# Varghese-Kuruvilla/Visual-Odometry-pipeline

Measured on NVIDIA B200. Metric: frame-pairs/sec (match+PnP), higher is better.
Workload: dtype tf32x3 / f32+f64 PnP

## Files before the change

### visual-odometry-pipeline_b200/csrc/match_f32_tc.cu

```cuda
#include "common.cuh"
#include "tc_ptx.cuh"
#include <cuda_fp16.h>
#include <stdlib.h>

#ifndef VO_TC_DBG
#define VO_TC_DBG 0
#endif
#ifndef VO_TC_PERSIST_MAX_TILES
#define VO_TC_PERSIST_MAX_TILES 64
#endif

namespace vo {
namespace {

constexpr int TC_BM = 128;
constexpr int TC_BN = 128;
constexpr int TC_D = 128;
constexpr int TC_KB = 32;
constexpr int TC_NKB = TC_D / TC_KB;
constexpr int TC_EXT_K = 8;
template <int PASSES>
struct TcCfg {
    static constexpr bool F8 = PASSES == 8 || PASSES == 9;
    static constexpr bool TOP1 = PASSES == 9;
    static constexpr bool K256 = F8;
    static constexpr bool F16 = PASSES == 16 || K256;
    static constexpr int KBOX = F8 ? 128 : 64;
    static constexpr bool H16 = F16 || PASSES == 48;
    static constexpr bool THREE = PASSES == 3 || PASSES == 48;
    static constexpr bool ALLWARP_COLS = PASSES == 48;
    static constexpr int KDIM = K256 ? 256 : TC_D;
    static constexpr bool SINGLE = !THREE;
    static constexpr int ALO = H16 ? 64 : TC_D;
    static constexpr int BN = F16 ? 192 : (SINGLE ? 160 : 128);
    static constexpr int STAGES = F16 ? 9 : (SINGLE ? 10 : 13);
    static constexpr int BLOCK_BYTES = BN * 128;
    static constexpr int TMEM_A = K256 ? 384 : (F16 ? 416 : (SINGLE ? 384 : 256));
    static constexpr int TMEM_EXT = F16 ? 384 : 320;
    static constexpr int OFF_SCOL = STAGES * BLOCK_BYTES;
    static constexpr int SCOL_N = F16 ? 0 : (ALLWARP_COLS ? 2 * 4 * BN : 2 * 2 * 4 * BN);
    static constexpr int OFF_ROW2 = OFF_SCOL + SCOL_N * 8;
    static constexpr int OFF_BAR = OFF_ROW2 + (H16 ? 4 * TC_BM * 4 : 0);
    static constexpr int SMEM_BYTES = OFF_BAR + 512 + 1024;
    static_assert(SMEM_BYTES <= 232448, "dynamic shared memory of one CTA (227 KB)");
    static constexpr uint32_t IDESC = (1u << 4) | (2u << 7) | (2u << 10) | ((uint32_t)(BN >> 3) << 17) | ((uint32_t)(TC_BM >> 4) << 24);
    static constexpr uint32_t IDESC16 = (1u << 4) | ((uint32_t)(BN >> 3) << 17) | ((uint32_t)(TC_BM >> 4) << 24);
    static constexpr float ACC_SCALE = PASSES == 48 ? 1.0f / 65536.0f : 1.0f;
};
constexpr int TC_THREADS = 576;
constexpr int TC_WARP_TMA = 16, TC_WARP_MMA = 17;
constexpr int TC_TMEM_COLS = 512;
constexpr int TC_CLUSTER = 2;

using namespace tc;



__global__ void __launch_bounds__(256)
prep_kernel(const float *__restrict__ x, long long rows, float *__restrict__ hi, float *__restrict__ lo,
            float *__restrict__ norm2, float *__restrict__ ext) {
    const long long row = (long long)blockIdx.x * 8 + (threadIdx.x >> 5);
    if (row >= rows) return;
    const int lane = threadIdx.x & 31;
    const float4 v = reinterpret_cast<const float4 *>(x)[row * 32 + lane];
    float4 h = make_float4(to_tf32(v.x), to_tf32(v.y), to_tf32(v.z), to_tf32(v.w));
    reinterpret_cast<float4 *>(hi)[row * 32 + lane] = h;
    if (lo) {
        float4 l = make_float4(to_tf32(v.x - h.x), to_tf32(v.y - h.y), to_tf32(v.z - h.z), to_tf32(v.w - h.w));
        reinterpret_cast<float4 *>(lo)[row * 32 + lane] = l;
    }
    if (norm2) {
        float s = __fadd_rn(__fadd_rn(__fmul_rn(v.x, v.x), __fmul_rn(v.y, v.y)), __fadd_rn(__fmul_rn(v.z, v.z), __fmul_rn(v.w, v.w)));
#pragma unroll
        for (int o = 16; o > 0; o >>= 1) s = __fadd_rn(s, __shfl_xor_sync(0xffffffffu, s, o));
        if (lane == 0) norm2[row] = s;
        if (ext) {
            float4 e = make_float4(0.f, 0.f, 0.f, 0.f);
            if (lane == 0) {
                const float n1 = to_tf32(s), n2 = to_tf32(__fsub_rn(s, n1));
                const float n3 = to_tf32(__fsub_rn(__fsub_rn(s, n1), n2));
                e = make_float4(-n1, -n2, -n3, 0.f);
            }
            if (lane < TC_EXT_K / 4) reinterpret_cast<float4 *>(ext)[row * (TC_EXT_K / 4) + lane] = e;
        }
    }
}

__global__ void __launch_bounds__(256)
prep16_kernel(const float *__restrict__ x, long long rows, __half *__restrict__ h16, float *__restrict__ norm2,
              float *__restrict__ ext) {
    const long long row = (long long)blockIdx.x * 8 + (threadIdx.x >> 5);
    if (row >= rows) return;
    const int lane = threadIdx.x & 31;
    const float4 v = reinterpret_cast<const float4 *>(x)[row * 32 + lane];
    const __half2 p0 = __floats2half2_rn(v.x, v.y), p1 = __floats2half2_rn(v.z, v.w);
    uint2 w;
    w.x = *reinterpret_cast<const uint32_t *>(&p0);
    w.y = *reinterpret_cast<const uint32_t *>(&p1);
    reinterpret_cast<uint2 *>(h16)[row * 32 + lane] = w;
    if (norm2) {
        float s = __fadd_rn(__fadd_rn(__fmul_rn(v.x, v.x), __fmul_rn(v.y, v.y)), __fadd_rn(__fmul_rn(v.z, v.z), __fmul_rn(v.w, v.w)));
#pragma unroll
        for (int o = 16; o > 0; o >>= 1) s = __fadd_rn(s, __shfl_xor_sync(0xffffffffu, s, o));
        if (lane == 0) norm2[row] = s;
        if (ext) {
// ... 193 lines not shown
                    s1 = gt ? sc[j0 + j] : s1;
                }
                thr = fmaxf(thr, s1);
            } else {
#pragma unroll
                for (int j = 0; j < 4; ++j) row_insert(sc[j0 + j], cbase + j0 + j, s1, s2, i1, i2);
                thr = fmaxf(thr, s2);
            }
        }
    }
}

template <bool EXT, bool F8>
__device__ __noinline__ void tc_a_to_tmem(const uint8_t *src, bool have, int k0, int row_elems, bool a_warp, bool ones_warp,
                                          uint32_t taddr_a, uint32_t taddr_ext, uint32_t bar_a, uint32_t wait_bar,
                                          uint32_t wait_parity, int lane) {
    constexpr int EPV = F8 ? 16 : 8;
    float v[32];
    if (a_warp) {
#pragma unroll
        for (int k = 0; k < 8; ++k) {
            uint4 x = (have && k0 + k * EPV < row_elems) ? __ldg(reinterpret_cast<const uint4 *>(src) + k) : make_uint4(0, 0, 0, 0);
            uint32_t wd[4] = {x.x, x.y, x.z, x.w};
#pragma unroll
            for (int i = 0; i < 4; ++i) {
                if (EXT) {
                    const __half2 d = __hmul2(*reinterpret_cast<const __half2 *>(&wd[i]), __floats2half2_rn(2.0f, 2.0f));
                    wd[i] = *reinterpret_cast<const uint32_t *>(&d);
                }
                v[4 * k + i] = __uint_as_float(wd[i]);
            }
        }
    }
    if (wait_bar) {
        tc::mbar_wait(wait_bar, wait_parity);
        tc::tc_fence_after();
    }
    if (a_warp) {
        tc::tc_st32(taddr_a, v);
        asm volatile("tcgen05.wait::st.sync.aligned;" ::: "memory");
        tc::tc_fence_before();
        if (lane == 0) tc::mbar_arrive(bar_a);
    }
    if (EXT && ones_warp) {
        const float ones[8] = {1.f, 1.f, 1.f, 0.f, 0.f, 0.f, 0.f, 0.f};
        tc::tc_st8(taddr_ext, ones);
        asm volatile("tcgen05.wait::st.sync.aligned;" ::: "memory");
        tc::tc_fence_before();
        if (lane == 0) tc::mbar_arrive(bar_a);
    }
}

template <int PASSES, int METRIC, bool COLS, bool PERSIST_T = false>
__global__ void __cluster_dims__(TC_CLUSTER, 1, 1) __launch_bounds__(TC_THREADS, 1)
match_f32_tc_kernel(const __grid_constant__ CUtensorMap map_b_hi, const __grid_constant__ CUtensorMap map_b_lo,
                    const float *__restrict__ a_hi, const float *__restrict__ a_lo, int n_stride, int m_stride,
                    const int32_t *__restrict__ n_ref, const int32_t *__restrict__ n_cur,
                    const float *__restrict__ row_norm, const float *__restrict__ col_norm, int n_split,
                    vo_row_partial *__restrict__ part, unsigned long long *__restrict__ colkey,
                    long long *__restrict__ dbg, int pair_group, int row_elems, int lgrid_x, int n_pairs) {
    extern __shared__ uint8_t smem_raw[];
    const uint32_t base = (smem_u32(smem_raw) + 1023u) & ~1023u;
    uint8_t *smem = smem_raw + (base - smem_u32(smem_raw));

    int b = blockIdx.z, rblock = blockIdx.x;
    if (pair_group > 1) {
        const int clusters_x = gridDim.x / TC_CLUSTER;
        const int set0 = (blockIdx.z / pair_group) * pair_group;
        const int gs = min(pair_group, (int)gridDim.z - set0);
        const int l = (blockIdx.z - set0) * clusters_x + (int)(blockIdx.x / TC_CLUSTER);
        b = set0 + l % gs;
        rblock = (l / gs) * TC_CLUSTER + (int)(blockIdx.x % TC_CLUSTER);
    }
    const int split = blockIdx.y;
    const int N = n_ref ? min(n_ref[b], n_stride) : n_stride;
    const int M = n_cur ? min(n_cur[b], m_stride) : m_stride;
    const int row0 = rblock * TC_BM;
    using Cfg = TcCfg<PASSES>;
    constexpr int BN = Cfg::BN, STAGES = Cfg::STAGES, BLOCK_BYTES = Cfg::BLOCK_BYTES, HALF = BN / 2;
    constexpr int TMEM_A = Cfg::TMEM_A, TMEM_EXT = Cfg::TMEM_EXT;
    constexpr uint32_t IDESC = Cfg::IDESC;
    const int tiles_total = (M + BN - 1) / BN;
    const int tiles_per_split = (tiles_total + n_split - 1) / n_split;
    const int t_begin = min(tiles_total, split * tiles_per_split);
    const int t_end = min(tiles_total, t_begin + tiles_per_split);
    const int n_tiles = t_end - t_begin;
    constexpr bool PERSIST = PERSIST_T;
    static_assert(!PERSIST || Cfg::F16, "only the fp16 / fp8 single passes have the item loop in their epilogue");
    struct Item { int b, row0, split, N, M, t_begin, n_tiles; };
    const int w_step = PERSIST ? (int)gridDim.x / TC_CLUSTER : 1;
    const int w_first = PERSIST ? (int)blockIdx.x / TC_CLUSTER : 0;
    const int w_end = PERSIST ? (lgrid_x / TC_CLUSTER) * n_split * n_pairs : 1;
    auto item_at = [&](int w) {
        Item I;
        if (!PERSIST) { I.b = b; I.row0 = row0; I.split = split; I.N = N; I.M = M; I.t_begin = t_begin; I.n_tiles = n_tiles; return I; }
        const int cx = lgrid_x / TC_CLUSTER;
        I.b = w / (cx * n_split);
        I.split = (w / cx) % n_split;
        I.row0 = ((w % cx) * TC_CLUSTER + (int)(blockIdx.x % TC_CLUSTER)) * TC_BM;
        I.N = n_ref ? min(n_ref[I.b], n_stride) : n_stride;
        I.M = n_cur ? min(n_cur[I.b], m_stride) : m_stride;
        const int tt = (I.M + BN - 1) / BN, tps = (tt + n_split - 1) / n_split;
        I.t_begin = min(tt, I.split * tps);
        I.n_tiles = min(tt, I.t_begin + tps) - I.t_begin;
        return I;
    };
    const int warp = threadIdx.x >> 5, lane = threadIdx.x & 31;
    const uint32_t crank = cluster_rank();
    const bool dbg_on = VO_TC_DBG && dbg != nullptr && rblock == 0 && blockIdx.y == 0 && b == 0;
    const long long t_kernel0 = dbg_on ? clock64() : 0;
    const bool trace_on = VO_TC_DBG && dbg != nullptr && dbg[15] == 1;
    const long long t_trace0 = (trace_on && threadIdx.x == 0) ? clock64() : 0;
#define TC_DBG_BEGIN() const long long _t0 = dbg_on ? clock64() : 0
#define TC_DBG_END(slot) do { if (dbg_on) dbg_acc[slot] += clock64() - _t0; } while (0)
    long long dbg_acc[4] = {0, 0, 0, 0};

    constexpr bool F16 = Cfg::F16;
    constexpr bool H16 = Cfg::H16, THREE = Cfg::THREE, SCALED = PASSES == 48;
    constexpr bool EXT = !THREE && (METRIC == VO_METRIC_L2);
    constexpr int NKB = H16 ? Cfg::KDIM / Cfg::KBOX : TC_NKB;
    constexpr int ITEMS = THREE ? 2 * NKB : (EXT ? NKB + 1 : NKB);
    const uint32_t s_b = base;
    float *scol_v = reinterpret_cast<float *>(smem + Cfg::OFF_SCOL);
    uint32_t *scol_b = reinterpret_cast<uint32_t *>(smem + Cfg::OFF_SCOL + Cfg::SCOL_N * 4);
    const uint32_t s_bar = base + Cfg::OFF_BAR;
    auto bar_full = [&](int s) { return s_bar + 8u * s; };
    auto bar_empty = [&](int s) { return s_bar + 8u * (STAGES + s); };
    const uint32_t bar_a = s_bar + 8u * (2 * STAGES);
    auto bar_tfull = [&](int g) { return s_bar + 8u * (2 * STAGES + 1 + g); };
    auto bar_tempty = [&](int g) { return s_bar + 8u * (2 * STAGES + 3 + g); };
    uint32_t *tmem_slot = reinterpret_cast<uint32_t *>(smem + Cfg::OFF_BAR + 8 * (2 * STAGES + 5));
    volatile float *srow2 = reinterpret_cast<volatile float *>(smem + Cfg::OFF_ROW2);
    if (Cfg::H16 && threadIdx.x < 4 * TC_BM) srow2[threadIdx.x] = -INFINITY;

    if (threadIdx.x == 0) {
        for (int s = 0; s < STAGES; ++s) {
            mbar_init(bar_full(s), 1);
            mbar_init(bar_empty(s), TC_CLUSTER);
        }
        mbar_init(bar_a, THREE ? 16 : (EXT ? 12 : 8));
        for (int g = 0; g < 2; ++g) { mbar_init(bar_tfull(g), 1); mbar_init(bar_tempty(g), H16 ? 16 : 8); }
        asm volatile("fence.mbarrier_init.release.cluster;" ::: "memory");
    }
    if (warp == TC_WARP_MMA) {
        asm volatile("tcgen05.alloc.cta_group::1.sync.aligned.shared::cta.b32 [%0], %1;" ::"r"(smem_u32(tmem_slot)),
                     "r"((uint32_t)TC_TMEM_COLS)
                     : "memory");
        asm volatile("tcgen05.relinquish_alloc_permit.cta_group::1.sync.aligned;" ::: "memory");
    }
    tc_fence_before();
    __syncthreads();
    cluster_sync_all();
    tc_fence_after();
    const uint32_t tmem_base = *tmem_slot;
    if (dbg_on && threadIdx.x == 0) dbg[14] = clock64() - t_kernel0;

    auto tile_of = [&](int lt) { return t_begin + lt; };

    if (warp == TC_WARP_TMA) {
        if (lane == 0) {
            int it = 0;
            for (int w = w_first; w < w_end; w += w_step) {
            const Item I = item_at(w);
            for (int lt = 0; lt < I.n_tiles; ++lt) {
                const int brow = I.b * m_stride + (I.t_begin + lt) * BN;
                for (int item = 0; item < ITEMS; ++item, ++it) {
                    const int stage = it % STAGES;
                    const uint32_t phase = (uint32_t)(it / STAGES) & 1u;
                    { TC_DBG_BEGIN(); mbar_wait(bar_empty(stage), phase ^ 1u); TC_DBG_END(0); }
                    const bool is_ext = EXT && item == NKB;
                    mbar_expect_tx(bar_full(stage), is_ext ? BN * TC_EXT_K * 4 : BLOCK_BYTES);
                    if ((uint32_t)(it & 1) == crank) {
                        const int kb = is_ext ? 0 : (THREE ? (item >> 1) : item);
                        const bool is_lo = is_ext || (THREE && (item & 1));
                        tma_load_2d_mc(s_b + stage * BLOCK_BYTES, is_lo ? &map_b_lo : &map_b_hi, kb * (H16 ? Cfg::KBOX : TC_KB), brow,
                                       bar_full(stage), (uint16_t)((1u << TC_CLUSTER) - 1u));
                    }
                }
            }
            }
            if (dbg_on) dbg[4] = dbg_acc[0];
        }
    } else if (warp == TC_WARP_MMA) {
        {
            uint32_t stage = 0, phase = 0, a_phase = 0;
            long long mma_wait_full = 0, mma_wait_tempty = 0, mma_wait_a = 0;
            int gt = 0;
            for (int w = w_first; w < w_end; w += w_step) {
            const Item I = item_at(w);
            if (I.n_tiles == 0) continue;
            { const long long _t0 = dbg_on ? clock64() : 0;
              mbar_wait(bar_a, a_phase);
              if (dbg_on) mma_wait_a += clock64() - _t0; }
            a_phase ^= 1u;
            tc_fence_after();
            for (int lt = 0; lt < I.n_tiles; ++lt, ++gt) {
                const int buf = gt & 1;
                const uint32_t use = (uint32_t)(gt >> 1);
                { const long long _t0 = dbg_on ? clock64() : 0;
                  mbar_wait(bar_tempty(buf), (use & 1u) ^ 1u);
                  if (dbg_on) mma_wait_tempty += clock64() - _t0; }
                tc_fence_after();
                const uint32_t d_tmem = tmem_base + (uint32_t)(buf * BN);
#pragma unroll
                for (int item = 0; item < ITEMS; ++item) {
                    { const long long _t0 = dbg_on ? clock64() : 0;
                      mbar_wait(bar_full(stage), phase);
                      if (dbg_on) mma_wait_full += clock64() - _t0; }
                    tc_fence_after();
                    if (elect_one()) {
                        const int kb = THREE ? (item >> 1) : item;
                        const bool is_lo = THREE && (item & 1);
                        const uint32_t b_lo32 = (((s_b + stage * BLOCK_BYTES) & 0x3ffffu) >> 4) | (1u << 16);
                        const uint32_t a_hi_t = tmem_base + (uint32_t)(TMEM_A + kb * TC_KB);
                        if (EXT && item == NKB) {
                            const uint64_t bdesc = ((uint64_t)TC_SDESC_HI_32B << 32) | (uint64_t)b_lo32;
                            tc_mma_tf32_ts(d_tmem, tmem_base + (uint32_t)TMEM_EXT, bdesc, IDESC, 1u);
                        } else
#pragma unroll
                        for (int k8 = 0; k8 < TC_KB / 8; ++k8) {
                            const uint64_t bdesc = ((uint64_t)TC_SDESC_HI << 32) | (uint64_t)(b_lo32 + k8 * 2);
                            const uint32_t ahi = a_hi_t + k8 * 8;
                            if (Cfg::F8) {
                                tc_mma_f8_ts(d_tmem, ahi, bdesc, Cfg::IDESC16, (item | k8) ? 1u : 0u);
                            } else if (F16) {
// ... 119 lines not shown
#undef TC_FOLD8
                srow2[cq * TC_BM + rr] = Cfg::TOP1 ? s1 : s2;
                if (edbg) dbg_acc[2] += clock64() - _tm0;
                ++gt;
            };
            for (int lt = 0; lt < n_t - 1; ++lt) tile(lt, false);
            if (n_t > 0) {
                bool waited = false;
                if (has_next) {
                    const Item Nx = item_at(w + w_step);
                    if (Nx.n_tiles > 0) {
                        a_put(Nx.b, Nx.row0, bar_tfull(gt & 1), (uint32_t)(gt >> 1) & 1u);
                        a_stored = waited = true;
                    }
                }
                tile(n_t - 1, waited);
            }
            if (edbg) t_between = clock64();
            if (METRIC == VO_METRIC_L2) {
                s1 = __fsub_rn(s1, na); s2 = __fsub_rn(s2, na);
            }
            {
                const Item I = item_at(w);
                if (I.row0 + rr < n_stride) {
                    const size_t at = ((size_t)I.b * (n_split * 4) + I.split * 4 + cq) * n_stride + I.row0 + rr;
                    if (Cfg::TOP1) {
                        vo_row_best q;
                        q.s1 = float_to_ordered(-s1); q.i1 = i1;
                        reinterpret_cast<vo_row_best *>(part)[at] = q;
                    } else {
                        vo_row_partial p;
                        p.s1 = float_to_ordered(-s1); p.s2 = float_to_ordered(-s2);
                        p.i1 = i1; p.i2 = i2;
                        part[at] = p;
                    }
                }
            }
            if (has_next) {
                srow2[cq * TC_BM + rr] = -INFINITY;
                asm volatile("bar.sync 1, 512;" ::: "memory");
            }
        }
        if (edbg && q == 0 && lane == 0 && cq < 2) { dbg[5 + cq] = dbg_acc[0]; dbg[7 + cq] = dbg_acc[1]; dbg[9 + cq] = dbg_acc[2]; if (cq == 1) dbg[13] = dbg_acc[3]; }
        } else if constexpr (Cfg::ALLWARP_COLS) {
        constexpr int QW = BN / 4;
        static_assert(QW == 32, "two 16-column reads per thread, one merged column per lane");
        const int cq = warp >> 2;
        const int q = warp & 3;
        const int row = row0 + q * 32 + lane;
        const bool row_ok = row < N;
        const bool partial_rows = row0 + TC_BM > N;
        const uint32_t lane_base = tmem_base + ((uint32_t)(q * 32) << 16);
        if (n_tiles > 0) {
            const __half *src = reinterpret_cast<const __half *>(cq < 2 ? a_hi : a_lo) +
                                ((size_t)b * n_stride + min(row, n_stride - 1)) * TC_D + (cq & 1) * 64;
            const bool have = row < n_stride;
            float v[32];
#pragma unroll
            for (int k = 0; k < 8; ++k) {
                const uint4 x = have ? __ldg(reinterpret_cast<const uint4 *>(src) + k) : make_uint4(0, 0, 0, 0);
                v[4 * k] = __uint_as_float(x.x); v[4 * k + 1] = __uint_as_float(x.y);
                v[4 * k + 2] = __uint_as_float(x.z); v[4 * k + 3] = __uint_as_float(x.w);
            }
            tc_st32(lane_base + (uint32_t)(TMEM_A + cq * 32), v);
            asm volatile("tcgen05.wait::st.sync.aligned;" ::: "memory");
            tc_fence_before();
            if (lane == 0) mbar_arrive(bar_a);
        }
        float s1 = -INFINITY, s2 = -INFINITY, thr = -INFINITY;
        int32_t i1 = -1, i2 = -1;
        const int rr = q * 32 + lane;
        const float *cn = (METRIC == VO_METRIC_L2) ? col_norm + (size_t)b * m_stride : nullptr;
        const float na = (METRIC == VO_METRIC_L2 && row_ok) ? row_norm[(size_t)b * n_stride + row] : 0.0f;
        const bool cn_vec = (METRIC == VO_METRIC_L2) && ((reinterpret_cast<uintptr_t>(cn) & 15u) == 0);
        for (int lt = 0; lt < n_tiles; ++lt) {
            const int buf = lt & 1;
            const uint32_t use = (uint32_t)(lt >> 1);
            const int tcol0 = tile_of(lt) * BN;
            const int col0 = tcol0 + cq * QW;
            const bool full_tile = tcol0 + BN <= M;
            float *tile_cv = scol_v + buf * 4 * BN;
            uint32_t *tile_cb = scol_b + buf * 4 * BN;
            float *my_cv = tile_cv + q * BN + cq * QW;
            uint32_t *my_cb = tile_cb + q * BN + cq * QW;
            { TC_DBG_BEGIN(); mbar_wait(bar_tfull(buf), use & 1u); TC_DBG_END(0); }
            tc_fence_after();
            const long long _tc0 = dbg_on ? clock64() : 0;
            const uint32_t taddr = lane_base + (uint32_t)(buf * BN + cq * QW);
            uint32_t ra[16], rb[16];
            tc_ld16_issue(taddr, ra);
            tc_ld16_issue(taddr + 16, rb);
            {
                const float tau = fmaxf(fmaxf(srow2[((cq + 1) & 3) * TC_BM + rr], srow2[((cq + 2) & 3) * TC_BM + rr]),
                                        srow2[((cq + 3) & 3) * TC_BM + rr]);
                thr = fmaxf(thr, row_threshold(s2, tau));
            }
            float colthr = -INFINITY;
            bool col_any = false;
            if (COLS) {
                const int c = col0 + lane;
                float cur_best = INFINITY;
                if (c < M) {
                    const unsigned long long key = *reinterpret_cast<const volatile unsigned long long *>(colkey + (size_t)b * m_stride + c);
                    cur_best = (key == ~0ull) ? -INFINITY : -ordered_to_float((uint32_t)(key >> 32));
                }
                colthr = -warp_max_f32(-cur_best);
                my_cb[lane] = 0u;
                __syncwarp();
            }
            tc_ld_wait16(ra);
            tc_ld_wait16(rb);
            tc_fence_before();
            if (lane == 0) mbar_arrive(bar_tempty(buf));
            if (dbg_on) dbg_acc[1] += clock64() - _tc0;
            const long long _tm0 = dbg_on ? clock64() : 0;
#define TC_FOLD16(BUF, J0, MASKC, MASKR)                                                                                   \
    _Pragma("unroll") for (int u = 0; u < 2; ++u) {                                                                        \
        float v[8];                                                                                                        \
        _Pragma("unroll") for (int i = 0; i < 8; ++i) v[i] = __uint_as_float(BUF[8 * u + i]);                              \
        epi_group8<METRIC, MASKC, MASKR, COLS, false, SCALED, true>(v, col0 + (J0) + 8 * u, M, row_ok, na, cn, cn_vec, lane, \
                                                                  my_cv + (J0) + 8 * u, my_cb + (J0) + 8 * u, s1, s2, i1,  \
                                                                  i2, thr, colthr, &col_any);                              \
    }
            if (full_tile && !partial_rows) {
                TC_FOLD16(ra, 0, false, false) TC_FOLD16(rb, 16, false, false)
            } else {
                TC_FOLD16(ra, 0, true, true) TC_FOLD16(rb, 16, true, true)
            }
#undef TC_FOLD16
            srow2[cq * TC_BM + rr] = s2;
            if (COLS) {
                uint32_t merge;
                asm volatile("{\n\t.reg .pred p, r;\n\tsetp.ne.u32 p, %1, 0;\n\tbar.red.or.pred r, %2, 128, p;\n\tselp.u32 %0, 1, 0, r;\n\t}"
                             : "=r"(merge)
                             : "r"((uint32_t)col_any), "r"(1 + cq)
                             : "memory");
                if (q == 0 && merge) {
                    const int j = cq * QW + lane;
                    const int col = tcol0 + j;
                    float best = -INFINITY;
                    int brow = -1;
#pragma unroll
                    for (int qq = 0; qq < 4; ++qq) {
                        const float val = tile_cv[qq * BN + j];
                        const uint32_t bal = tile_cb[qq * BN + j];
                        if (bal != 0u && val > best) { best = val; brow = qq * 32 + __ffs(bal) - 1; }
                    }
                    if (col < M && brow >= 0 && row0 + brow < N) {
                        const unsigned long long key =
                            ((unsigned long long)float_to_ordered(-best) << 32) | (unsigned long long)(uint32_t)(row0 + brow);
                        unsigned long long *dst = colkey + (size_t)b * m_stride + col;
                        if (key < *reinterpret_cast<volatile unsigned long long *>(dst)) atomicMin(dst, key);
                    }
                }
            }
            if (dbg_on) dbg_acc[2] += clock64() - _tm0;
        }
        if (dbg_on && q == 0 && lane == 0 && cq < 2) { dbg[5 + cq] = dbg_acc[0]; dbg[7 + cq] = dbg_acc[1]; dbg[9 + cq] = dbg_acc[2]; }
        if (METRIC == VO_METRIC_L2 && !COLS) {
            s1 = __fsub_rn(s1, na); s2 = __fsub_rn(s2, na);
        }
        if (row < n_stride) {
            vo_row_partial p;
            p.s1 = float_to_ordered(-s1); p.s2 = float_to_ordered(-s2);
            p.i1 = i1; p.i2 = i2;
            part[((size_t)b * (n_split * 4) + split * 4 + cq) * n_stride + row] = p;
        }
        } else {
        const int g = warp >> 3;
        const int h = (warp >> 2) & 1;
        const int q = warp & 3;
        const int row = row0 + q * 32 + lane;
        const bool row_ok = row < N;
        const bool partial_rows = row0 + TC_BM > N;
        const uint32_t lane_base = tmem_base + ((uint32_t)(q * 32) << 16);

        if (n_tiles > 0 && (g == 0 || THREE)) {
            const float *src = (g == 0 ? a_hi : a_lo) + ((size_t)b * n_stride + min(row, n_stride - 1)) * TC_D;
            const bool have = row < n_stride;
#pragma unroll 1
            for (int c = 2 * h; c < 2 * h + 2; ++c) {
                float v[32];
#pragma unroll
                for (int k = 0; k < 8; ++k) {
                    const float4 x = have ? __ldg(reinterpret_cast<const float4 *>(src + c * 32) + k) : make_float4(0, 0, 0, 0);
                    const float sc2 = EXT ? 2.0f : 1.0f;
                    v[4 * k] = sc2 * x.x; v[4 * k + 1] = sc2 * x.y; v[4 * k + 2] = sc2 * x.z; v[4 * k + 3] = sc2 * x.w;
                }
                tc_st32(lane_base + (uint32_t)(TMEM_A + g * TC_D + c * 32), v);
            }
            asm volatile("tcgen05.wait::st.sync.aligned;" ::: "memory");
            tc_fence_before();
            if (lane == 0) mbar_arrive(bar_a);
        }

        if (EXT && n_tiles > 0 && g == 1 && h == 0) {
            const float ones[8] = {1.f, 1.f, 1.f, 0.f, 0.f, 0.f, 0.f, 0.f};
            tc_st8(lane_base + (uint32_t)TMEM_EXT, ones);
            asm volatile("tcgen05.wait::st.sync.aligned;" ::: "memory");
            tc_fence_before();
            if (lane == 0) mbar_arrive(bar_a);
        }

        float s1 = -INFINITY, s2 = -INFINITY;
        float thr = -INFINITY;
        int32_t i1 = -1, i2 = -1;
        float *grp_cv = scol_v + g * 2 * 4 * BN;
        uint32_t *grp_cb = scol_b + g * 2 * 4 * BN;
        const float *cn = (METRIC == VO_METRIC_L2) ? col_norm + (size_t)b * m_stride : nullptr;
        const float na = (METRIC == VO_METRIC_L2 && row_ok) ? row_norm[(size_t)b * n_stride + row] : 0.0f;
        const bool cn_vec = (METRIC == VO_METRIC_L2) && ((reinterpret_cast<uintptr_t>(cn) & 15u) == 0);

        for (int lt = g; lt < n_tiles; lt += 2) {
            const int col0 = tile_of(lt) * BN;
            const uint32_t use = (uint32_t)(lt >> 1);
            const bool full_tile = col0 + BN <= M;
            float *tile_cv = grp_cv + (use & 1u) * 4 * BN;
            uint32_t *tile_cb = grp_cb + (use & 1u) * 4 * BN;
            float *my_cv = tile_cv + q * BN;
            uint32_t *my_cb = tile_cb + q * BN;
            { TC_DBG_BEGIN(); mbar_wait(bar_tfull(g), use & 1u); TC_DBG_END(0); }
            tc_fence_after();
            const long long _tc0 = dbg_on ? clock64() : 0;
            const uint32_t taddr = lane_base + (uint32_t)(g * BN);
            if (THREE) {
#define TC_EPI_LOOP(MASKC, MASKR)                                                                                          \
    _Pragma("unroll 1") for (int j0 = HALF * h; j0 < HALF * h + HALF; j0 += 8) {                                                 \
        uint32_t cur[8];                                                                                                   \
        tc_ld8_issue(taddr + j0, cur);                                                                                     \
        tc_ld_wait8(cur);                                                                                                  \
        float v[8];                                                                                                        \
        _Pragma("unroll") for (int i = 0; i < 8; ++i) v[i] = __uint_as_float(cur[i]);                                      \
        epi_group8<METRIC, MASKC, MASKR, COLS, EXT, SCALED>(v, col0 + j0, M, row_ok, na, cn, cn_vec, lane, my_cv + j0, my_cb + j0, \
                                                    s1, s2, i1, i2, thr);                                                       \
    }
                if (full_tile && !partial_rows) { TC_EPI_LOOP(false, false) } else { TC_EPI_LOOP(true, true) }
#undef TC_EPI_LOOP
            } else if (COLS) {
                uint32_t cur[8], nxt[8];
                tc_ld8_issue(taddr + HALF * h, cur);
                tc_ld_wait8(cur);
#define TC_EPI_LOOP(MASKC, MASKR)                                                                                          \
    _Pragma("unroll 1") for (int j0 = HALF * h; j0 < HALF * h + HALF; j0 += 8) {                                                 \
        const bool more = j0 + 8 < HALF * h + HALF;                                                                            \
        if (more) tc_ld8_issue(taddr + j0 + 8, nxt);                                                                       \
        float v[8];                                                                                                        \
        _Pragma("unroll") for (int i = 0; i < 8; ++i) v[i] = __uint_as_float(cur[i]);                                      \
        epi_group8<METRIC, MASKC, MASKR, COLS, EXT>(v, col0 + j0, M, row_ok, na, cn, cn_vec, lane, my_cv + j0, my_cb + j0, \
                                                    s1, s2, i1, i2, thr);                                                       \
        if (more) {                                                                                                        \
            tc_ld_wait8(nxt);                                                                                              \
            _Pragma("unroll") for (int i = 0; i < 8; ++i) cur[i] = nxt[i];                                                 \
        }                                                                                                                  \
    }
                if (full_tile && !partial_rows) { TC_EPI_LOOP(false, false) } else { TC_EPI_LOOP(true, true) }
#undef TC_EPI_LOOP
            } else {
                uint32_t bufa[16], bufb[16];
                tc_ld16_issue(taddr + HALF * h, bufa);
                tc_ld_wait16(bufa);
#define TC_FOLD16(BUF, J0, MASKC, MASKR)                                                                                   \
    _Pragma("unroll") for (int u = 0; u < 2; ++u) {                                                                        \
        float v[8];                                                                                                        \
        _Pragma("unroll") for (int i = 0; i < 8; ++i) v[i] = __uint_as_float(BUF[8 * u + i]);                              \
        epi_group8<METRIC, MASKC, MASKR, COLS, EXT>(v, col0 + (J0) + 8 * u, M, row_ok, na, cn, cn_vec, lane,               \
                                                    my_cv + (J0) + 8 * u, my_cb + (J0) + 8 * u, s1, s2, i1, i2, thr);           \
    }
#define TC_EPI_LOOP(MASKC, MASKR)                                                                                          \
    _Pragma("unroll 1") for (int j0 = HALF * h; j0 < HALF * h + HALF; j0 += 32) {                                          \
        const bool has_b = j0 + 16 < HALF * h + HALF;                  \
        if (has_b) tc_ld16_issue(taddr + j0 + 16, bufb);                                                                   \
        TC_FOLD16(bufa, j0, MASKC, MASKR)                                                                                  \
        if (has_b) {                                                                                                       \
            tc_ld_wait16(bufb);                                                                                            \
            const bool more = j0 + 32 < HALF * h + HALF;                                                                   \
            if (more) tc_ld16_issue(taddr + j0 + 32, bufa);                                                                \
            TC_FOLD16(bufb, j0 + 16, MASKC, MASKR)                                                                         \
            if (more) tc_ld_wait16(bufa);                                                                                  \
        }                                                                                                                  \
    }
                if (full_tile && !partial_rows) { TC_EPI_LOOP(false, false) } else { TC_EPI_LOOP(true, true) }
#undef TC_EPI_LOOP
#undef TC_FOLD16
            }
            tc_fence_before();
            if (lane == 0) mbar_arrive(bar_tempty(g));
            if (dbg_on) dbg_acc[1] += clock64() - _tc0;
            const long long _tm0 = dbg_on ? clock64() : 0;
            if (COLS) group_bar(1 + g);
            if (COLS && (h * 4 + q) * 32 < BN) {
                const int j = (h * 4 + q) * 32 + lane;
// ... 22 lines not shown
        if (row < n_stride) {
            vo_row_partial p;
            p.s1 = float_to_ordered(-s1); p.s2 = float_to_ordered(-s2);
            p.i1 = i1; p.i2 = i2;
            part[((size_t)b * (n_split * 4) + split * 4 + g * 2 + h) * n_stride + row] = p;
        }
        }
    }

    if (dbg_on && threadIdx.x == 0) dbg[0] = clock64() - t_kernel0;
    tc_fence_before();
    __syncthreads();
    cluster_sync_all();
    if (warp == TC_WARP_MMA) {
        asm volatile("tcgen05.dealloc.cta_group::1.sync.aligned.b32 %0, %1;" ::"r"(tmem_base), "r"((uint32_t)TC_TMEM_COLS)
                     : "memory");
    }
    if (trace_on && threadIdx.x == 0) {
        uint32_t smid;
        asm volatile("mov.u32 %0, %%smid;" : "=r"(smid));
        long long *t = dbg + 16 + 3 * ((size_t)(blockIdx.z * gridDim.y + blockIdx.y) * gridDim.x + blockIdx.x);
        t[0] = t_trace0; t[1] = clock64(); t[2] = smid;
    }
}

typedef CUresult (*PFN_encodeTiled)(CUtensorMap *, CUtensorMapDataType, cuuint32_t, void *, const cuuint64_t *,
                                    const cuuint64_t *, const cuuint32_t *, const cuuint32_t *, CUtensorMapInterleave,
                                    CUtensorMapSwizzle, CUtensorMapL2promotion, CUtensorMapFloatOOBfill);

int make_map(vo_ctx *ctx, CUtensorMap *map, const void *ptr, long long rows, int box_rows, int row_elems = TC_D,
             bool half = false, bool bytes = false, bool narrow = false) {
    PFN_encodeTiled fn = (PFN_encodeTiled)ctx->encode_tiled;
    const size_t esz = bytes ? 1 : (half ? 2 : 4);
    cuuint64_t dims[2] = {(cuuint64_t)row_elems, (cuuint64_t)rows};
    cuuint64_t strides[1] = {(cuuint64_t)row_elems * esz};
    cuuint32_t box[2] = {(cuuint32_t)((narrow ? 32 : 128) / esz), (cuuint32_t)box_rows};
    cuuint32_t estr[2] = {1, 1};
    CUresult r = fn(map, bytes ? CU_TENSOR_MAP_DATA_TYPE_UINT8 : (half ? CU_TENSOR_MAP_DATA_TYPE_FLOAT16 : CU_TENSOR_MAP_DATA_TYPE_FLOAT32), 2, (void *)ptr, dims, strides, box, estr,
                    CU_TENSOR_MAP_INTERLEAVE_NONE, narrow ? CU_TENSOR_MAP_SWIZZLE_32B : CU_TENSOR_MAP_SWIZZLE_128B, CU_TENSOR_MAP_L2_PROMOTION_L2_256B,
                    CU_TENSOR_MAP_FLOAT_OOB_FILL_NONE);
    if (r != CUDA_SUCCESS) {
        set_error("cuTensorMapEncodeTiled failed (CUresult %d)", (int)r);
        return VO_ERR_CUDA;
    }
    return VO_OK;
}

template <int PASSES, int METRIC, bool COLS, bool PERSIST>
int launch_tc_kern(vo_ctx *ctx, dim3 grid, const CUtensorMap &bh, const CUtensorMap &bl, const float *a_hi, const float *a_lo,
                   int n_stride, int m_stride, const int32_t *n_ref, const int32_t *n_cur, const float *row_norm,
                   const float *col_norm, int n_split, vo_row_partial *part, unsigned long long *colkey, cudaStream_t st,
                   int row_elems) {
    auto kern = match_f32_tc_kernel<PASSES, METRIC, COLS, PERSIST>;
    long long *dbg = nullptr;
    const size_t n_ctas = (size_t)grid.x * grid.y * grid.z;
    const bool trace = getenv("VO_TC_TRACE") != nullptr;
    if (VO_TC_DBG && (getenv("VO_TC_DEBUG") || trace)) {
        static long long *dbg_dev = nullptr;
        static size_t dbg_cap = 0;
        const size_t need = 16 + (trace ? 3 * n_ctas : 0);
        if (dbg_cap < need) {
            if (dbg_dev) VO_CUDA(cudaFree(dbg_dev));
            VO_CUDA(cudaMalloc(&dbg_dev, need * sizeof(long long)));
            dbg_cap = need;
        }
        VO_CUDA(cudaMemsetAsync(dbg_dev, 0, 16 * sizeof(long long), st));
        if (trace) {
            const long long one = 1;
            VO_CUDA(cudaMemcpyAsync(dbg_dev + 15, &one, sizeof(one), cudaMemcpyHostToDevice, st));
        }
        dbg = dbg_dev;
    }
    VO_CUDA(cudaFuncSetAttribute(kern, cudaFuncAttributeMaxDynamicSharedMemorySize, TcCfg<PASSES>::SMEM_BYTES));
    int pair_group = 1;
    if (TcCfg<PASSES>::ALLWARP_COLS && COLS && !getenv("VO_TC_NO_INTERLEAVE"))
        pair_group = (int)max(1ll, min(8ll, (64ll << 20) / ((long long)m_stride * TC_D * 4)));
    dim3 launch_grid = grid;
    if (PERSIST) {
        static int max_clusters = 0;
        if (max_clusters == 0) {
            cudaLaunchConfig_t cfg = {};
            cfg.gridDim = dim3(TC_CLUSTER * 64);
            cfg.blockDim = dim3(TC_THREADS);
            cfg.dynamicSmemBytes = TcCfg<PASSES>::SMEM_BYTES;
            cudaLaunchAttribute at;
            at.id = cudaLaunchAttributeClusterDimension;
            at.val.clusterDim.x = TC_CLUSTER; at.val.clusterDim.y = 1; at.val.clusterDim.z = 1;
            cfg.attrs = &at;
            cfg.numAttrs = 1;
            int n = 0;
            if (cudaOccupancyMaxActiveClusters(&n, kern, &cfg) != cudaSuccess || n <= 0) {
                (void)cudaGetLastError();
                n = ctx->sm_count / TC_CLUSTER;
            }
            max_clusters = n;
        }
        const long long items = (long long)(grid.x / TC_CLUSTER) * grid.y * grid.z;
        const long long clusters = items < max_clusters ? items : (long long)max_clusters;
        launch_grid = dim3((unsigned)(clusters * TC_CLUSTER), 1, 1);
    }
    kern<<<launch_grid, TC_THREADS, TcCfg<PASSES>::SMEM_BYTES, st>>>(bh, bl, a_hi, a_lo, n_stride, m_stride, n_ref, n_cur, row_norm, col_norm,
                                                  n_split, part, colkey, dbg, pair_group, row_elems, (int)grid.x, (int)grid.z);
    VO_LAUNCH_CHECK(ctx);
    if (dbg && trace) {
        VO_CUDA(cudaStreamSynchronize(st));
        long long *h = (long long *)malloc(3 * n_ctas * sizeof(long long));
        VO_CUDA(cudaMemcpy(h, dbg + 16, 3 * n_ctas * sizeof(long long), cudaMemcpyDeviceToHost));
        double busy = 0, gap = 0;
        long long n_gap = 0, max_gap = 0;
        for (int sm = 0; sm < 256; ++sm) {
            long long last_end = -1;
            for (;;) {
                long long best = -1;
                size_t bi = 0;
                for (size_t i = 0; i < n_ctas; ++i)
                    if (h[3 * i + 2] == sm && (last_end < 0 || h[3 * i] >= last_end) && (best < 0 || h[3 * i] < best)) {
                        best = h[3 * i];
                        bi = i;
                    }
                if (best < 0) break;
                if (last_end >= 0) { gap += (double)(best - last_end); ++n_gap; if (best - last_end > max_gap) max_gap = best - last_end; }
                busy += (double)(h[3 * bi + 1] - h[3 * bi]);
                last_end = h[3 * bi + 1];
            }
        }
        fprintf(stderr, "[vo tc trace] passes=%d ctas=%zu mean_cta_cycles=%.0f mean_gap_cycles=%.0f max_gap=%lld gaps=%lld\n", PASSES,
                n_ctas, busy / (double)n_ctas, n_gap ? gap / (double)n_gap : 0.0, max_gap, n_gap);
        free(h);
    } else if (dbg) {
// ... 53 lines not shown
    int rc;
    const bool f16 = passes == 16, h16 = passes == 16 || passes == 48, three = passes == 3 || passes == 48;
    const size_t esz = h16 ? sizeof(__half) : sizeof(float);
    const int row_elems = src_u8 ? src_u8 : TC_D;
    const bool ext = !three && l2;
    const size_t src_row_bytes = src_u8 ? (size_t)src_u8 : TC_D * sizeof(float);
    const bool chained = n_stride == m_stride && (n_stride & 3) == 0 && B > 0 && !getenv("VO_NO_CHAIN_PREP") &&
                         reinterpret_cast<const char *>(cur) == reinterpret_cast<const char *>(ref) + (size_t)n_stride * src_row_bytes;
    const long long rows_p = chained ? rows_a + n_stride : rows_a;
    const size_t per_a = (size_t)rows_p * row_elems * esz, per_b = chained ? 0 : (size_t)rows_b * row_elems * esz;
    if ((rc = ws_get(ctx, WS_SPLIT_A, per_a * (three ? 2 : 1), (void **)&split_a))) return rc;
    const size_t per_ext = (size_t)(chained ? rows_p : rows_b) * TC_EXT_K * sizeof(float);
    if ((rc = ws_get(ctx, WS_SPLIT_B, per_b * (three ? 2 : 1) + (ext ? per_ext : 0) + 16, (void **)&split_b))) return rc;
    const long long rows_a4 = (rows_a + 3) & ~3ll;
    if ((rc = ws_get(ctx, WS_NORMS, sizeof(float) * (size_t)(chained ? rows_p : rows_a4 + rows_b), (void **)&norms))) return rc;
    const size_t shift = (size_t)n_stride * row_elems * esz;
    float *a_hi = split_a, *a_lo = three ? reinterpret_cast<float *>(reinterpret_cast<char *>(split_a) + per_a) : nullptr;
    float *b_hi = chained ? reinterpret_cast<float *>(reinterpret_cast<char *>(a_hi) + shift) : split_b;
    float *b_lo = !three ? nullptr : (chained ? reinterpret_cast<float *>(reinterpret_cast<char *>(a_lo) + shift)
                                              : reinterpret_cast<float *>(reinterpret_cast<char *>(split_b) + per_b));
    float *x_ext = ext ? reinterpret_cast<float *>(reinterpret_cast<char *>(split_b) + per_b * (three ? 2 : 1)) : nullptr;
    float *b_ext = (ext && chained) ? x_ext + (size_t)n_stride * TC_EXT_K : x_ext;
    float *row_norm = norms, *col_norm = chained ? norms + n_stride : norms + rows_a4;

    VO_PROF(ctx, st, VO_STAGE_PREP);
    for (int side = 0; side < (chained ? 1 : 2); ++side) {
        const float *src = side ? cur : ref;
        const long long rows = side ? rows_b : rows_p;
        float *hi = side ? b_hi : a_hi, *lo = side ? b_lo : a_lo;
        float *nrm = l2 ? (side ? col_norm : row_norm) : nullptr;
        float *xe = (side || chained) ? x_ext : nullptr;
        const unsigned g8 = (unsigned)((rows + 7) / 8);
        if (passes == 48)
            prep16x3_kernel<<<g8, 256, 0, st>>>(src, rows, reinterpret_cast<__half *>(hi), reinterpret_cast<__half *>(lo), nrm);
        else if (f16 && src_u8 == 32)
            prep16_u8_kernel<32><<<(unsigned)((rows + 31) / 32), 256, 0, st>>>(reinterpret_cast<const uint8_t *>(src), rows, reinterpret_cast<__half *>(hi), side ? col_norm : row_norm, xe);
        else if (f16 && src_u8)
            prep16_u8_kernel<128><<<g8, 256, 0, st>>>(reinterpret_cast<const uint8_t *>(src), rows, reinterpret_cast<__half *>(hi), side ? col_norm : row_norm, xe);
        else if (f16)
            prep16_kernel<<<g8, 256, 0, st>>>(src, rows, reinterpret_cast<__half *>(hi), nrm, xe);
        else
            prep_kernel<<<g8, 256, 0, st>>>(src, rows, hi, lo, nrm, xe);
        VO_LAUNCH_CHECK(ctx);
    }

    CUtensorMap mbh, mbl;
    const int bn = three ? TcCfg<3>::BN : (f16 ? TcCfg<16>::BN : TcCfg<1>::BN);
    if ((rc = make_map(ctx, &mbh, b_hi, rows_b, bn, row_elems, h16))) return rc;
    if (ext) rc = make_map(ctx, &mbl, b_ext, rows_b, bn, TC_EXT_K, false, false, true);
    else rc = make_map(ctx, &mbl, three ? b_lo : b_hi, rows_b, bn, TC_D, h16);
    if (rc) return rc;

    const int row_blocks = ceil_div(n_stride, TC_BM);
    const int grid_x = ceil_div(row_blocks, TC_CLUSTER) * TC_CLUSTER;
    const int n_split = pick_split(ctx, B, grid_x, ceil_div(m_stride, bn), 4);
    vo_row_partial *part;
    if ((rc = ws_get(ctx, WS_ROWPART, sizeof(vo_row_partial) * (size_t)B * n_split * 4 * n_stride, (void **)&part))) return rc;
    dim3 grid(grid_x, n_split, B);
    VO_PROF(ctx, st, VO_STAGE_MATCH);
#define TC_ARGS ctx, grid, mbh, mbl, a_hi, a_lo, n_stride, m_stride, n_ref, n_cur, row_norm, col_norm, n_split, part, colkey, st
#define TC_PICK(P, MET) (need_cols ? launch_tc<P, MET, true>(TC_ARGS) : launch_tc<P, MET, false>(TC_ARGS))
    if (passes == 3) rc = l2 ? TC_PICK(3, VO_METRIC_L2) : TC_PICK(3, VO_METRIC_COSINE);
    else if (passes == 48) rc = l2 ? TC_PICK(48, VO_METRIC_L2) : TC_PICK(48, VO_METRIC_COSINE);
    else if (f16) rc = l2 ? launch_tc<16, VO_METRIC_L2, false>(TC_ARGS, row_elems) : launch_tc<16, VO_METRIC_COSINE, false>(TC_ARGS);
    else rc = l2 ? TC_PICK(1, VO_METRIC_L2) : TC_PICK(1, VO_METRIC_COSINE);
#undef TC_PICK
#undef TC_ARGS
    if (rc) return rc;
    *part_out = part;
    *n_split_out = n_split * 4;
    *row_norm_out = nullptr;
    return VO_OK;
}

int match_bits_tc(vo_ctx *ctx, const uint8_t *ref, const uint8_t *cur, int B, int n_stride, int m_stride, const int32_t *n_ref,
                  const int32_t *n_cur, int need_cols, int need_second, vo_row_partial **part_out, int *n_split_out,
                  unsigned long long *colkey, cudaStream_t st) {
    if (!ctx->tc_ready) {
        void *fn = nullptr;
        cudaDriverEntryPointQueryResult qres;
        VO_CUDA(cudaGetDriverEntryPoint("cuTensorMapEncodeTiled", &fn, cudaEnableDefault, &qres));
        if (qres != cudaDriverEntryPointSuccess || !fn) {
            set_error("cuTensorMapEncodeTiled is not available from this driver");
            return VO_ERR_UNSUPPORTED;
        }
        ctx->encode_tiled = fn;
        ctx->tc_ready = 1;
    }
    constexpr int KD = 256, BN = TcCfg<8>::BN;
    const long long rows_a = (long long)B * n_stride, rows_b = (long long)B * m_stride;
    uint8_t *a8, *b8;
    int rc;
    const bool chained = n_stride == m_stride && B > 0 && !getenv("VO_NO_CHAIN_PREP") && cur == ref + (size_t)n_stride * 32;
    const long long rows_p = chained ? rows_a + n_stride : rows_a;
    if ((rc = ws_get(ctx, WS_SPLIT_A, (size_t)rows_p * KD, (void **)&a8))) return rc;
    if (chained) b8 = a8 + (size_t)n_stride * KD;
    else if ((rc = ws_get(ctx, WS_SPLIT_B, (size_t)rows_b * KD, (void **)&b8))) return rc;
    VO_PROF(ctx, st, VO_STAGE_PREP);
    prep_bits8_kernel<<<(unsigned)((rows_p + 7) / 8), 256, 0, st>>>(ref, rows_p, a8);
    VO_LAUNCH_CHECK(ctx);
    if (!chained) {
        prep_bits8_kernel<<<(unsigned)((rows_b + 7) / 8), 256, 0, st>>>(cur, rows_b, b8);
        VO_LAUNCH_CHECK(ctx);
    }

    auto pass = [&](const uint8_t *A, const uint8_t *Bm, int ns, int ms, const int32_t *na, const int32_t *nb, int slot,
                    vo_row_partial **part, int *n_split, bool second) -> int {
        CUtensorMap map;
        int r;
        if ((r = make_map(ctx, &map, Bm, (long long)B * ms, BN, KD, false, true))) return r;
        const int row_blocks = ceil_div(ns, TC_BM);
        const int grid_x = ceil_div(row_blocks, TC_CLUSTER) * TC_CLUSTER;
        const int ns_split = pick_split(ctx, B, grid_x, ceil_div(ms, BN), 4);
        if ((r = ws_get(ctx, slot, sizeof(vo_row_partial) * (size_t)B * ns_split * 4 * ns, (void **)part))) return r;
        dim3 grid(grid_x, ns_split, B);
        *n_split = ns_split * 4;
        if (second)
            return launch_tc<8, VO_METRIC_COSINE, false>(ctx, grid, map, map, reinterpret_cast<const float *>(A), nullptr, ns, ms, na, nb,
                                                         nullptr, nullptr, ns_split, *part, nullptr, st, KD);
        return launch_tc<9, VO_METRIC_COSINE, false>(ctx, grid, map, map, reinterpret_cast<const float *>(A), nullptr, ns, ms, na, nb,
                                                     nullptr, nullptr, ns_split, *part, nullptr, st, KD);
    };
    VO_PROF(ctx, st, VO_STAGE_MATCH);
    if ((rc = pass(a8, b8, n_stride, m_stride, n_ref, n_cur, WS_ROWPART, part_out, n_split_out, need_second != 0))) return rc;
    if (need_cols) {
        vo_row_partial *part2;
        int n_split2;
        if ((rc = pass(b8, a8, m_stride, n_stride, n_cur, n_ref, WS_ROWPART2, &part2, &n_split2, false))) return rc;
        colkey_from_partials_kernel<<<dim3(ceil_div(m_stride, 256), B), 256, 0, st>>>(reinterpret_cast<const vo_row_best *>(part2), n_split2,
                                                                                      m_stride, n_cur, colkey);
        VO_LAUNCH_CHECK(ctx);
    }
    return VO_OK;
}

}
```

Before: 8371.

## Use 4-CTA TMA multicast clusters and all-warp epilogue for 3-pass TF32 matching

For the 3-pass (tf32x3) matcher, the thread-block cluster grows from 2 to 4 CTAs, so each B tile is loaded once by one CTA and multicast to four, cutting L2 traffic per CTA. The 3-pass path also moves to the all-warp epilogue with the A-fill layout generalized to fp32 chunks, and the interleave pair_group sizing now accounts for element width. Larger clusters can make scheduling harder, can pad more row blocks per pair, and make every stage slot wait for more consumers before it is freed.

```diff
diff --git a/visual-odometry-pipeline_b200/csrc/match_f32_tc.cu b/visual-odometry-pipeline_b200/csrc/match_f32_tc.cu
--- a/visual-odometry-pipeline_b200/csrc/match_f32_tc.cu
+++ b/visual-odometry-pipeline_b200/csrc/match_f32_tc.cu
@@ -5,6 +5,9 @@
 
 #ifndef VO_TC_DBG
 #define VO_TC_DBG 0
+#endif
+#ifndef VO_TC_CLUSTER3
+#define VO_TC_CLUSTER3 4
 #endif
 #ifndef VO_TC_PERSIST_MAX_TILES
 #define VO_TC_PERSIST_MAX_TILES 64
@@ -28,7 +31,8 @@
     static constexpr int KBOX = F8 ? 128 : 64;
     static constexpr bool H16 = F16 || PASSES == 48;
     static constexpr bool THREE = PASSES == 3 || PASSES == 48;
-    static constexpr bool ALLWARP_COLS = PASSES == 48;
+    static constexpr bool ALLWARP_COLS = THREE;
+    static constexpr bool ALLWARP = F16 || ALLWARP_COLS;
     static constexpr int KDIM = K256 ? 256 : TC_D;
     static constexpr bool SINGLE = !THREE;
     static constexpr int ALO = H16 ? 64 : TC_D;
@@ -40,17 +44,17 @@
     static constexpr int OFF_SCOL = STAGES * BLOCK_BYTES;
     static constexpr int SCOL_N = F16 ? 0 : (ALLWARP_COLS ? 2 * 4 * BN : 2 * 2 * 4 * BN);
     static constexpr int OFF_ROW2 = OFF_SCOL + SCOL_N * 8;
-    static constexpr int OFF_BAR = OFF_ROW2 + (H16 ? 4 * TC_BM * 4 : 0);
+    static constexpr int OFF_BAR = OFF_ROW2 + (ALLWARP ? 4 * TC_BM * 4 : 0);
     static constexpr int SMEM_BYTES = OFF_BAR + 512 + 1024;
     static_assert(SMEM_BYTES <= 232448, "dynamic shared memory of one CTA (227 KB)");
     static constexpr uint32_t IDESC = (1u << 4) | (2u << 7) | (2u << 10) | ((uint32_t)(BN >> 3) << 17) | ((uint32_t)(TC_BM >> 4) << 24);
     static constexpr uint32_t IDESC16 = (1u << 4) | ((uint32_t)(BN >> 3) << 17) | ((uint32_t)(TC_BM >> 4) << 24);
     static constexpr float ACC_SCALE = PASSES == 48 ? 1.0f / 65536.0f : 1.0f;
+    static constexpr int CLUSTER = PASSES == 3 ? VO_TC_CLUSTER3 : 2;
 };
 constexpr int TC_THREADS = 576;
 constexpr int TC_WARP_TMA = 16, TC_WARP_MMA = 17;
 constexpr int TC_TMEM_COLS = 512;
-constexpr int TC_CLUSTER = 2;
 
 using namespace tc;
 
@@ -350,7 +354,7 @@
 }
 
 template <int PASSES, int METRIC, bool COLS, bool PERSIST_T = false>
-__global__ void __cluster_dims__(TC_CLUSTER, 1, 1) __launch_bounds__(TC_THREADS, 1)
+__global__ void __cluster_dims__(TcCfg<PASSES>::CLUSTER, 1, 1) __launch_bounds__(TC_THREADS, 1)
 match_f32_tc_kernel(const __grid_constant__ CUtensorMap map_b_hi, const __grid_constant__ CUtensorMap map_b_lo,
                     const float *__restrict__ a_hi, const float *__restrict__ a_lo, int n_stride, int m_stride,
                     const int32_t *__restrict__ n_ref, const int32_t *__restrict__ n_cur,
@@ -358,6 +362,7 @@
                     vo_row_partial *__restrict__ part, unsigned long long *__restrict__ colkey,
                     long long *__restrict__ dbg, int pair_group, int row_elems, int lgrid_x, int n_pairs) {
     extern __shared__ uint8_t smem_raw[];
+    constexpr int TC_CLUSTER = TcCfg<PASSES>::CLUSTER;
     const uint32_t base = (smem_u32(smem_raw) + 1023u) & ~1023u;
     uint8_t *smem = smem_raw + (base - smem_u32(smem_raw));
 
@@ -429,7 +434,7 @@
     auto bar_tempty = [&](int g) { return s_bar + 8u * (2 * STAGES + 3 + g); };
     uint32_t *tmem_slot = reinterpret_cast<uint32_t *>(smem + Cfg::OFF_BAR + 8 * (2 * STAGES + 5));
     volatile float *srow2 = reinterpret_cast<volatile float *>(smem + Cfg::OFF_ROW2);
-    if (Cfg::H16 && threadIdx.x < 4 * TC_BM) srow2[threadIdx.x] = -INFINITY;
+    if (Cfg::ALLWARP && threadIdx.x < 4 * TC_BM) srow2[threadIdx.x] = -INFINITY;
 
     if (threadIdx.x == 0) {
         for (int s = 0; s < STAGES; ++s) {
@@ -437,7 +442,7 @@
             mbar_init(bar_empty(s), TC_CLUSTER);
         }
         mbar_init(bar_a, THREE ? 16 : (EXT ? 12 : 8));
-        for (int g = 0; g < 2; ++g) { mbar_init(bar_tfull(g), 1); mbar_init(bar_tempty(g), H16 ? 16 : 8); }
+        for (int g = 0; g < 2; ++g) { mbar_init(bar_tfull(g), 1); mbar_init(bar_tempty(g), Cfg::ALLWARP ? 16 : 8); }
         asm volatile("fence.mbarrier_init.release.cluster;" ::: "memory");
     }
     if (warp == TC_WARP_MMA) {
@@ -468,7 +473,7 @@
                     { TC_DBG_BEGIN(); mbar_wait(bar_empty(stage), phase ^ 1u); TC_DBG_END(0); }
                     const bool is_ext = EXT && item == NKB;
                     mbar_expect_tx(bar_full(stage), is_ext ? BN * TC_EXT_K * 4 : BLOCK_BYTES);
-                    if ((uint32_t)(it & 1) == crank) {
+                    if ((uint32_t)it % TC_CLUSTER == crank) {
                         const int kb = is_ext ? 0 : (THREE ? (item >> 1) : item);
                         const bool is_lo = is_ext || (THREE && (item & 1));
                         tma_load_2d_mc(s_b + stage * BLOCK_BYTES, is_lo ? &map_b_lo : &map_b_hi, kb * (H16 ? Cfg::KBOX : TC_KB), brow,
@@ -694,17 +699,22 @@
         const bool partial_rows = row0 + TC_BM > N;
         const uint32_t lane_base = tmem_base + ((uint32_t)(q * 32) << 16);
         if (n_tiles > 0) {
-            const __half *src = reinterpret_cast<const __half *>(cq < 2 ? a_hi : a_lo) +
-                                ((size_t)b * n_stride + min(row, n_stride - 1)) * TC_D + (cq & 1) * 64;
+            constexpr int CHUNKS = H16 ? 1 : 2;
+            static_assert(Cfg::ALO == 2 * CHUNKS * 32, "A_lo follows A_hi: quarter cq stores TMEM columns (cq * CHUNKS + c) * 32");
+            const uint8_t *src = reinterpret_cast<const uint8_t *>(cq < 2 ? a_hi : a_lo) +
+                                 ((size_t)b * n_stride + min(row, n_stride - 1)) * TC_D * (H16 ? 2 : 4) + (cq & 1) * CHUNKS * 128;
             const bool have = row < n_stride;
-            float v[32];
-#pragma unroll
-            for (int k = 0; k < 8; ++k) {
-                const uint4 x = have ? __ldg(reinterpret_cast<const uint4 *>(src) + k) : make_uint4(0, 0, 0, 0);
-                v[4 * k] = __uint_as_float(x.x); v[4 * k + 1] = __uint_as_float(x.y);
-                v[4 * k + 2] = __uint_as_float(x.z); v[4 * k + 3] = __uint_as_float(x.w);
-            }
-            tc_st32(lane_base + (uint32_t)(TMEM_A + cq * 32), v);
+#pragma unroll 1
+            for (int c = 0; c < CHUNKS; ++c) {
+                float v[32];
+#pragma unroll
+                for (int k = 0; k < 8; ++k) {
+                    const uint4 x = have ? __ldg(reinterpret_cast<const uint4 *>(src + c * 128) + k) : make_uint4(0, 0, 0, 0);
+                    v[4 * k] = __uint_as_float(x.x); v[4 * k + 1] = __uint_as_float(x.y);
+                    v[4 * k + 2] = __uint_as_float(x.z); v[4 * k + 3] = __uint_as_float(x.w);
+                }
+                tc_st32(lane_base + (uint32_t)(TMEM_A + (cq * CHUNKS + c) * 32), v);
+            }
             asm volatile("tcgen05.wait::st.sync.aligned;" ::: "memory");
             tc_fence_before();
             if (lane == 0) mbar_arrive(bar_a);
@@ -809,6 +819,7 @@
             part[((size_t)b * (n_split * 4) + split * 4 + cq) * n_stride + row] = p;
         }
         } else {
+        static_assert(PASSES == 1, "the other passes run an all-warp epilogue");
         const int g = warp >> 3;
         const int h = (warp >> 2) & 1;
         const int q = warp & 3;
@@ -817,8 +828,8 @@
         const bool partial_rows = row0 + TC_BM > N;
         const uint32_t lane_base = tmem_base + ((uint32_t)(q * 32) << 16);
 
-        if (n_tiles > 0 && (g == 0 || THREE)) {
-            const float *src = (g == 0 ? a_hi : a_lo) + ((size_t)b * n_stride + min(row, n_stride - 1)) * TC_D;
+        if (n_tiles > 0 && g == 0) {
+            const float *src = a_hi + ((size_t)b * n_stride + min(row, n_stride - 1)) * TC_D;
             const bool have = row < n_stride;
 #pragma unroll 1
             for (int c = 2 * h; c < 2 * h + 2; ++c) {
@@ -829,7 +840,7 @@
                     const float sc2 = EXT ? 2.0f : 1.0f;
                     v[4 * k] = sc2 * x.x; v[4 * k + 1] = sc2 * x.y; v[4 * k + 2] = sc2 * x.z; v[4 * k + 3] = sc2 * x.w;
                 }
-                tc_st32(lane_base + (uint32_t)(TMEM_A + g * TC_D + c * 32), v);
+                tc_st32(lane_base + (uint32_t)(TMEM_A + c * 32), v);
             }
             asm volatile("tcgen05.wait::st.sync.aligned;" ::: "memory");
             tc_fence_before();
@@ -865,20 +876,7 @@
             tc_fence_after();
             const long long _tc0 = dbg_on ? clock64() : 0;
             const uint32_t taddr = lane_base + (uint32_t)(g * BN);
-            if (THREE) {
-#define TC_EPI_LOOP(MASKC, MASKR)                                                                                          \
-    _Pragma("unroll 1") for (int j0 = HALF * h; j0 < HALF * h + HALF; j0 += 8) {                                                 \
-        uint32_t cur[8];                                                                                                   \
-        tc_ld8_issue(taddr + j0, cur);                                                                                     \
-        tc_ld_wait8(cur);                                                                                                  \
-        float v[8];                                                                                                        \
-        _Pragma("unroll") for (int i = 0; i < 8; ++i) v[i] = __uint_as_float(cur[i]);                                      \
-        epi_group8<METRIC, MASKC, MASKR, COLS, EXT, SCALED>(v, col0 + j0, M, row_ok, na, cn, cn_vec, lane, my_cv + j0, my_cb + j0, \
-                                                    s1, s2, i1, i2, thr);                                                       \
-    }
-                if (full_tile && !partial_rows) { TC_EPI_LOOP(false, false) } else { TC_EPI_LOOP(true, true) }
-#undef TC_EPI_LOOP
-            } else if (COLS) {
+            if (COLS) {
                 uint32_t cur[8], nxt[8];
                 tc_ld8_issue(taddr + HALF * h, cur);
                 tc_ld_wait8(cur);
@@ -1007,6 +1005,7 @@
                    const float *col_norm, int n_split, vo_row_partial *part, unsigned long long *colkey, cudaStream_t st,
                    int row_elems) {
     auto kern = match_f32_tc_kernel<PASSES, METRIC, COLS, PERSIST>;
+    constexpr int TC_CLUSTER = TcCfg<PASSES>::CLUSTER;
     long long *dbg = nullptr;
     const size_t n_ctas = (size_t)grid.x * grid.y * grid.z;
     const bool trace = getenv("VO_TC_TRACE") != nullptr;
@@ -1028,8 +1027,10 @@
     }
     VO_CUDA(cudaFuncSetAttribute(kern, cudaFuncAttributeMaxDynamicSharedMemorySize, TcCfg<PASSES>::SMEM_BYTES));
     int pair_group = 1;
-    if (TcCfg<PASSES>::ALLWARP_COLS && COLS && !getenv("VO_TC_NO_INTERLEAVE"))
-        pair_group = (int)max(1ll, min(8ll, (64ll << 20) / ((long long)m_stride * TC_D * 4)));
+    if (TcCfg<PASSES>::ALLWARP_COLS && COLS && !getenv("VO_TC_NO_INTERLEAVE")) {
+        const long long b_row_bytes = 2ll * TC_D * (TcCfg<PASSES>::H16 ? 2 : 4);
+        pair_group = (int)max(1ll, min(8ll, (64ll << 20) / ((long long)m_stride * b_row_bytes)));
+    }
     dim3 launch_grid = grid;
     if (PERSIST) {
         static int max_clusters = 0;
@@ -1189,7 +1190,8 @@
     if (rc) return rc;
 
     const int row_blocks = ceil_div(n_stride, TC_BM);
-    const int grid_x = ceil_div(row_blocks, TC_CLUSTER) * TC_CLUSTER;
+    const int cluster = passes == 3 ? TcCfg<3>::CLUSTER : 2;
+    const int grid_x = ceil_div(row_blocks, cluster) * cluster;
     const int n_split = pick_split(ctx, B, grid_x, ceil_div(m_stride, bn), 4);
     vo_row_partial *part;
     if ((rc = ws_get(ctx, WS_ROWPART, sizeof(vo_row_partial) * (size_t)B * n_split * 4 * n_stride, (void **)&part))) return rc;
@@ -1247,7 +1249,7 @@
         int r;
         if ((r = make_map(ctx, &map, Bm, (long long)B * ms, BN, KD, false, true))) return r;
         const int row_blocks = ceil_div(ns, TC_BM);
-        const int grid_x = ceil_div(row_blocks, TC_CLUSTER) * TC_CLUSTER;
+        const int grid_x = ceil_div(row_blocks, TcCfg<8>::CLUSTER) * TcCfg<8>::CLUSTER;
         const int ns_split = pick_split(ctx, B, grid_x, ceil_div(ms, BN), 4);
         if ((r = ws_get(ctx, slot, sizeof(vo_row_partial) * (size_t)B * ns_split * 4 * ns, (void **)part))) return r;
         dim3 grid(grid_x, ns_split, B);
```

New measurement: 8001 (median of 6 runs). 0.956x the previous value.
